# IDSIA/hhmarl_2D

Hardware: AMD Instinct MI355X
Metric: env-steps/sec (2v2) (higher is better)
Workload: dtype f64

## Files before the change

### hhmarl_2d_amd/csrc/hh_kernels_quad.h

```cpp
#ifndef HH_KERNELS_QUAD_H
#define HH_KERNELS_QUAD_H

#include "hh_kernels.h"

#define HH_QP(a, b, c, d) ((a) | ((b) << 2) | ((c) << 4) | ((d) << 6))

template <int CTRL>
__device__ __forceinline__ int q_perm_i(int v) { return __builtin_amdgcn_mov_dpp(v, CTRL, 0xf, 0xf, true); }
template <int CTRL>
__device__ __forceinline__ float q_perm_f(float v) { return __int_as_float(q_perm_i<CTRL>(__float_as_int(v))); }
template <int CTRL>
__device__ __forceinline__ double q_perm_d(double v) {
    int lo = __double2loint(v), hi = __double2hiint(v);
    lo = q_perm_i<CTRL>(lo);
    hi = q_perm_i<CTRL>(hi);
    return __hiloint2double(hi, lo);
}
#define HH_QROT(K) HH_QP((K) & 3, ((K) + 1) & 3, ((K) + 2) & 3, ((K) + 3) & 3)
template <int K> __device__ __forceinline__ int q_rot_i(int v) { return q_perm_i<HH_QROT(K)>(v); }
template <int K> __device__ __forceinline__ float q_rot_f(float v) { return q_perm_f<HH_QROT(K)>(v); }
template <int K> __device__ __forceinline__ double q_rot_d(double v) { return q_perm_d<HH_QROT(K)>(v); }
template <int J> __device__ __forceinline__ int q_bc_i(int v) { return q_perm_i<HH_QP(J, J, J, J)>(v); }
template <int J> __device__ __forceinline__ double q_bc_d(double v) { return q_perm_d<HH_QP(J, J, J, J)>(v); }
__device__ __forceinline__ double q_mate_d(double v) { return q_perm_d<HH_QP(1, 0, 3, 2)>(v); }
// ... 14 lines not shown

struct QPub {
    double uc, us, un;
    float nlat, nlon, nspd, nhdg;
    int flags;
};

struct QTab {
    double lat[3], lon[3];
    double dist[3], foc[3], focr[3], hd[3];
    float nlat[3], nlon[3], nspd[3], nhdg[3];
    int fl[3];
    int amask;
};

__device__ __forceinline__ void quad_publish_vec(const Unit &m, QPub &p) {
    double sn, cs;
    hh_sincos(hh_pymod360(90.0 - m.hdg) * (HH_PI / 180.0), &sn, &cs);
    p.uc = cs;
    p.us = sn;
    p.un = hh_sqrt(cs * cs + sn * sn);
}
__device__ __forceinline__ void quad_publish_norm(const DevCfg &c, const Unit &m, QPub &p) {
    p.nlat = (float)hh_clip(hh_div_known(m.lat - HH_MAP_LAT0, c.ext_lat, c.inv_ext_lat), 0.0, 1.0);
    p.nlon = (float)hh_clip(hh_div_known(m.lon - HH_MAP_LON0, c.ext_lon, c.inv_ext_lon), 0.0, 1.0);
    p.nspd = (float)hh_clip(hh_div_known(m.spd, HH_AC_MAX_SPEED(m.ac_type), HH_AC_INV_MAX_SPEED(m.ac_type)), 0.0, 1.0);
    p.nhdg = (float)hh_clip(HH_DIVC(hh_pymod359(m.hdg), 359.0), 0.0, 1.0);
}
__device__ __forceinline__ void quad_publish_motion(const DevCfg &c, const Unit &m, QPub &p) {
    quad_publish_vec(m, p);
    quad_publish_norm(c, m, p);
}

struct QPosMail { double lat[64], lon[64], spd[64], hdg[64]; int ac_type[64], steps[64], episode[64], escw[64]; };
struct QTabMail { double dist[3][64], foc[3][64], focr[3][64]; double uc[64], us[64], sx[64], sy[64]; unsigned long long tk[64];
                  double sp_hdg[64], sp_spd[64]; int sp_w[64];
                  double nr0[64], nfoc[64], nfocr[64]; int nbw[64]; };
struct QTgt { double foc, focr, dist; };
struct QSlimMail { int flags[64], w5[64], w6[64], w7[64]; double rew[64]; int full; };
struct QAheadMail { double u[2][64]; };
struct QPre {
    bool ok;
    bool a_ok;
    int a_par;
    bool spec;
    double sp_hdg, sp_spd;
    int sp_w;
    unsigned long long tkey;
    double sx, sy;
};
__device__ __forceinline__ void quad_publish_flags(const Unit &m, QPub &p) {
    int shot = m.burst > 0 || (m.ac_type == 1 && m.has_missile);
    p.flags = (m.alive ? FL_ALIVE : 0) | ((m.ac_type & 3) << 1) | (shot ? FL_SHOT : 0);
}
__device__ __forceinline__ void quad_publish(const DevCfg &c, const Unit &m, QPub &p) {
    quad_publish_motion(c, m, p);
    quad_publish_flags(m, p);
}

__device__ __forceinline__ void quad_tables_obs(const QPub &p, int s, QTab &t) {
#define HH_QFETCHO(K)                                                                 \
    t.nlat[K - 1] = q_rot_f<K>(p.nlat); t.nlon[K - 1] = q_rot_f<K>(p.nlon);               \
    t.nspd[K - 1] = q_rot_f<K>(p.nspd); t.nhdg[K - 1] = q_rot_f<K>(p.nhdg);               \
    t.fl[K - 1] = q_rot_i<K>(p.flags);
    HH_QFETCHO(1)
    HH_QFETCHO(2)
    HH_QFETCHO(3)
// ... 131 lines not shown
        }
        n += quad_opp_block(t, 0, nb.k0, nb.d0, out + n);
    } else {
        out[n++] = (float)hh_clip((double)m.cannon_remain / (double)m.cannon_max, 0.0, 1.0);
        if (m.ac_type == 1) out[n++] = (float)hh_clip((double)m.missile_remain / (double)m.rocket_max, 0.0, 1.0);
        out[n++] = (p.flags & FL_SHOT) ? 1.0f : 0.0f;
        quad_opp_block(t, 1, nb.k0, nb.d0, out + n);
        if (nb.n >= 2) quad_opp_block(t, 1, nb.k1, nb.d1, out + n + 9);
        else for (int k = 0; k < 9; k++) out[n + 9 + k] = 0.0f;
        n += 18;
    }
    const int kf = ((s ^ 1) - s) & 3;
    if ((t.amask >> (s ^ 1)) & 1) {
        out[n++] = q_sel(t.nlat, kf);
        out[n++] = q_sel(t.nlon, kf);
        out[n++] = (float)norm180(q_sel(t.foc, kf));
        out[n++] = (float)norm180(q_sel(t.focr, kf));
        out[n++] = (float)(c.inv_diag * q_sel(t.dist, kf));
    } else {
        for (int k = 0; k < 5; k++) out[n++] = 0.0f;
    }
}

__device__ __forceinline__ bool q_any(bool x) {
    unsigned long long b = __ballot(x);
    asm volatile("" : "+s"(b));
    return b != 0ULL;
}

__device__ __forceinline__ void arm_cannon_if(Unit &m, bool cond) {
    const int b = HH_AC_BURST(m.ac_type);
    const int armed = m.cannon_remain < b ? m.cannon_remain : b;
    m.burst = cond ? armed : m.burst;
}

__device__ __forceinline__ void q_wave_sync() { asm volatile("s_waitcnt lgkmcnt(0)" ::: "memory"); }

__device__ __forceinline__ void quad_l3_flags(int steps, unsigned long long tkey, int amask0, int s, int &esc, int &esc_t, bool &my_escaping, bool (&escj)[2]) {
    const bool draw_tick = steps % 60 == 0;
    const bool any_draw = q_any(draw_tick);
#pragma unroll
    for (int j = 2; j < 4; j++) {
        const bool aj = ((amask0 >> j) & 1) != 0;
        if (HH_RARE(any_draw)) {
            if (aj & draw_tick & (esc == 0)) {
                esc = hh_rng_randint(hh_rng_u01(tkey, (uint32_t)(j + 1), HH_SITE_L3_ESC_COIN, 0u), 0, 1);
                if (esc) esc_t = (int)hh_rng_uniform(hh_rng_u01(tkey, (uint32_t)(j + 1), HH_SITE_L3_ESC_TIME, 0u), 20.0, 30.0);
            }
        }
        const bool mine = aj & (j == s), upd = aj & (esc != 0);
        my_escaping = mine ? (esc != 0) : my_escaping;
        escj[j - 2] = aj & (esc != 0);
        const int esc_t1 = esc_t - 1;
        esc_t = upd ? esc_t1 : esc_t;
        esc = (upd & (esc_t <= 0)) ? 0 : esc;
    }
}
struct QScriptOut { double heading, speed; int fire, fire_m, opp; };
__device__ __forceinline__ void quad_l3_script(const DevCfg &c, double lat, double lon, double hdg, int ac_type, bool my_escaping, double u0, double u1, double u2,
                                               const Near2 &nb, const QTab &tb, double focus_k0, double rs, double rc, QScriptOut &o) {
    int opp = -1, fire = 0, fire_m = 0;
    double heading, speed;
    if (my_escaping) {
        double y = hh_clip(hh_div_known(lat - HH_MAP_LAT0, c.ext_lat, c.inv_ext_lat), 0.0, 1.0);
        double x = hh_clip(hh_div_known(lon - HH_MAP_LON0, c.ext_lon, c.inv_ext_lon), 0.0, 1.0);
        double uh = u0;
        double lo_h = y < 0.5 ? (x < 0.5 ? 30.0 : 300.0) : (x < 0.5 ? 120.0 : 210.0);
        heading = (double)(int)hh_rng_uniform(uh, lo_h, lo_h + 30.0);
        speed = (double)(int)hh_rng_uniform(u1, 300.0, 600.0);
        fire = hh_rng_randint(u2, 0, 1);
    } else {
        heading = hdg;
        speed = (double)(int)hh_rng_uniform(u0, 100.0, 400.0);
        if (nb.n) {
            const double ag_lat = q_sel(tb.lat, nb.k0), ag_lon = q_sel(tb.lon, nb.k0);
            double x1 = lon + rs, y1 = lat + rc;
            double val = (x1 - lon) * (ag_lat - lat) - (ag_lon - lon) * (y1 - lat);
            double sign = val < 0.0 ? 1.0 : -1.0;
            double r = hh_rng_uniform(u1, 0.7, 1.3);
            double focus = focus_k0;
            const double turned = hh_pymod360(heading + r * sign * focus);
            heading = ((nb.d0 > 0.008) & (focus > 4.0)) ? turned : heading;
            const double us = u2;
            const double sp_near = (double)(int)hh_rng_uniform(us, 500.0, 800.0), sp_far = (double)(int)hh_rng_uniform(us, 100.0, 500.0);
            const double sp2 = focus < 30.0 ? sp_near : sp_far;
            speed = nb.d0 > 0.05 ? sp2 : speed;
            fire = nb.d0 < 0.03 && focus < 10.0;
            fire_m = nb.d0 < 0.09 && focus < 5.0;
            opp = nb.j0;
        }
        if (ac_type == 2) speed = hh_clip(speed, 0.0, 600.0);
    }
    if (heading >= 360.0 || heading < 0.0) heading = 0.0;
    o.heading = heading; o.speed = speed; o.fire = fire; o.fire_m = fire_m; o.opp = opp;
}

template <bool IX, bool DUAL, bool OWT = false>
__device__ __forceinline__ void tick_quad(const DevCfg &c, Shared<4, 64> &sh, int tid, int g, int s, int base, bool active, bool helper, Unit &m,
                                          Arena &ar, const int8_t *act, QTab &tb, QPub &pub, Near2 &nbc, const QTgt &tg, StepOut &out,
                                          uint32_t &ev_mask_out, QPosMail *pos, const QAheadMail *ahd, const QPre &pre HH_PROF_ARGS) {
    constexpr int A = 4;
    const int id = s + 1;
    const bool running = active & (ar.done == 0);
    const bool agent = s < 2;
    out.reward = 0.0;
    out.valid = 0;
    out.kill_event = 0;
    uint32_t evm = 0;
    {
        const int steps1 = ar.steps + 1;
        ar.steps = running ? steps1 : ar.steps;
        if (OWT && HH_USUAL(pre.ok)) ar.tkey = running ? pre.tkey : ar.tkey;
        else if (running) arena_rekey(ar);
    }
    const bool snap = running & (m.alive != 0);
    const int amask0 = tb.amask;
    const int rk_age0 = (m.rk_alive && m.rk_life <= HH_ROCKET_MAX_LIFE) ? m.rk_life : 0;
    const double rk_speed0 = sh.rk_speed[rk_age0];
    const int tgt_at_act = m.n_tgt ? m.tgt0 : 0;
    int want_launch = 0, launch_tgt = 0;
    int wait_after = -1;
    bool base_gate = false;
    constexpr bool AHEAD = OWT && DUAL;
    double u_noise_ahead = 0.0;
    if constexpr (AHEAD) u_noise_ahead = ahd->u[pre.a_par][tid & 31];
    const bool a_ok = AHEAD && pre.a_ok;

    {
        if (HH_USUAL(snap & (agent | (c.ext_opp != 0)))) {
            int t = m.n_tgt ? m.tgt0 : 0;
            if (!agent) {
                const Near2 nb = nbc;
                m.n_tgt = nb.n ? 1 : 0; m.tgt0 = nb.n ? nb.j0 + 1 : 0; m.tgt_d0 = nb.n ? nb.d0 : 0.0;
                t = m.tgt0;
            }
            out.valid = agent ? 1 : out.valid;
#ifdef HHQ_ABL_DECODE
            m.cmd_hdg = m.hdg; m.cmd_spd = 300.0;
#else
            const double nh = hh_pymod360(m.hdg + (double)(((int)act[0] - 6) * 15));
            const bool nh_out = (nh >= 360.0) | (nh < 0.0);
            m.cmd_hdg = nh_out ? 0.0 : nh;
            double mx = HH_AC_MAX_SPEED(m.ac_type);
            m.cmd_spd = 100.0 + ((mx - 100.0) / 8.0) * (double)act[1];
#endif
            {
                const bool arm = (act[2] != 0) & (m.cannon_remain > 0);
                arm_cannon_if(m, arm);
                const double rw = out.reward - 0.1;
                const bool pen = arm & agent & (c.agent_mode == HH_MODE_ESCAPE) & (m.cannon_remain < 90);
                out.reward = pen ? rw : out.reward;
            }
            {
                const bool gate = (m.ac_type == 1) & (act[3] != 0) & (t != 0) & (m.missile_remain > 0) & (m.has_missile == 0) & (m.missile_wait == 0);
                base_gate = gate;
                want_launch = gate ? 1 : want_launch;
                launch_tgt = gate ? t - 1 : launch_tgt;
            }
        } else if (snap && c.level <= 2) {
            if (c.level == 2) {
                arm_cannon(m);
                bool man = ar.steps <= 5;
                if (!man) man = (ar.steps % hh_rng_randint(d_rng(ar, id, HH_SITE_L2_PERIOD, 0), 35, 45)) <= 5;
                if (man) {
                    int r = hh_rng_randint(d_rng(ar, id, HH_SITE_L2_TURN, 0), 0, 1);
                    m.cmd_hdg = hh_pymod360(m.hdg + (r ? -90.0 : 90.0));
                    m.cmd_spd = (double)(100 + hh_rng_randint(d_rng(ar, id, HH_SITE_L2_SPEED, 0), 0, 4) * 75);
                }
            }
            if (!m.has_missile && (ar.steps % 40) < 3 && hh_rng_randint(d_rng(ar, id, HH_SITE_L12_COIN, 0), 0, 1) &&
                m.missile_wait == 0 && m.ac_type == 1) {
                const Near2 nb = nbc;
                if (nb.n) { want_launch = 1; launch_tgt = nb.j0; wait_after = 5; }
            }
        }
    }
    HH_PROF(11);
    const bool spec = OWT && pre.ok && pre.spec && !c.ext_opp && c.level >= 3;
    bool my_escaping = false;
    bool escj[2] = {false, false};
    if (HH_RARE(!spec)) {
    if (HH_USUAL(running && !c.ext_opp && c.level >= 3)) {
        int esc = ar.escaping, esc_t = ar.escaping_time;
        quad_l3_flags(ar.steps, ar.tkey, amask0, s, esc, esc_t, my_escaping, escj);
        ar.escaping = esc;
        ar.escaping_time = esc_t;
    }
    double u0 = 0.0, u1 = 0.0, u2 = 0.0;
    if (!c.ext_opp && c.level >= 3) {
        {
            const int du = (s | 2) + 1;
            const bool desc = (s & 1) ? escj[1] : escj[0];
// ... 137 lines not shown
#else
            d_geo_move(x_lat, x_lon, x_hdg, x_s, o_lat, o_lon);
#endif
            m.lat = mv_a ? o_lat : m.lat; m.lon = mv_a ? o_lon : m.lon;
            rk_nlat = q_up_d(o_lat); rk_nlon = q_up_d(o_lon);
        } else if (HH_USUAL(any_rk)) {
            const double r_spd = rk_speed0;
            double a_lat, a_lon;
            d_geo_move2(m.lat, m.lon, m.hdg, mv_a ? m.spd * HH_KNOTS_TO_MS * 1.0 : 0.0, a_lat, a_lon,
                        rk_spec ? r_lat : 5.0, rk_spec ? r_lon : 7.0, r_hdg, r_spd * HH_KNOTS_TO_MS * 1.0, rk_nlat, rk_nlon);
            m.lat = mv_a ? a_lat : m.lat; m.lon = mv_a ? a_lon : m.lon;
        } else {
            if (mv_a) d_geo_move(m.lat, m.lon, m.hdg, m.spd * HH_KNOTS_TO_MS * 1.0, m.lat, m.lon);
        }
    }
    const double rk0_lat = rk_pre ? m.rk_lat : lat_old, rk0_lon = rk_pre ? m.rk_lon : lon_old;
    QPub pn;
    if constexpr (OWT) {
        {
            const double th = turn_deg * (HH_PI / 180.0), t2 = th * th;
            const double cd = 1.0 + t2 * (-0.5 + t2 * (1.0 / 24.0));
            const double sd = th * (1.0 + t2 * ((-1.0 / 6.0) + t2 * (1.0 / 120.0)));
            pn.uc = pub.uc * cd + pub.us * sd;
            pn.us = pub.us * cd - pub.uc * sd;
            pn.un = 1.0;
        }
        pn.nlat = pn.nlon = pn.nspd = pn.nhdg = 0.0f;
        pos->lat[tid] = m.lat;
        pos->lon[tid] = m.lon;
        pos->spd[tid] = m.spd; pos->hdg[tid] = m.hdg; pos->ac_type[tid] = m.ac_type;
        pos->steps[tid] = ar.steps; pos->episode[tid] = ar.episode;
        pos->escw[tid] = (ar.escaping & 0xff) | ((ar.escaping_time & 0xff) << 8) | ((amask0 & 0xf) << 16);
        HH_PROF(1);
        __syncthreads();
        HH_PROF(12);
    } else {
        quad_publish_motion(c, m, pn);
    }
    double lat1[3], lon1[3];
    lat1[0] = q_rot_d<1>(m.lat); lon1[0] = q_rot_d<1>(m.lon);
    lat1[1] = q_rot_d<2>(m.lat); lon1[1] = q_rot_d<2>(m.lon);
    lat1[2] = q_rot_d<3>(m.lat); lon1[2] = q_rot_d<3>(m.lon);

    HH_PROF(1);
    const int rk_tgt = rk_pre ? m.rk_target - 1 : launch_tgt;
    const bool rk_maybe = running && (rk_pre || try_launch);
    int launch_pre = -1;
    if (q_any(try_launch)) {
        const int kl = (launch_tgt - s) & 3;
        const double t_lat = q_sel(tb.lat, kl), t_lon = q_sel(tb.lon, kl);
        const double cross = pub.uc * (t_lat - lat_old) - pub.us * (t_lon - lon_old);
        const int lp = hh_missile_cone_planar(lat_old, lon_old, t_lat, t_lon, OWT ? tg.foc : q_sel(tb.foc, kl), cross, OWT ? tg.dist : q_sel(tb.dist, kl));
        launch_pre = try_launch ? lp : -1;
    }
    int q_total = 0;
    {
        int push[6];
        int code[6];
        push[0] = try_launch && launch_pre < 0;
        code[0] = tid | (0 << 8) | (launch_tgt << 10);
        const int t = m.ac_type;
#pragma unroll
        for (int k = 1; k < A; k++) {
            const int j = (s + k) & 3;
            const bool snap_j = running && ((amask0 >> j) & 1);
            const bool enemy = (j >= 2) != (s >= 2);
            const double tl = j < s ? lat1[k - 1] : tb.lat[k - 1];
// ... 3 lines not shown
#else
            push[k] = (int)fired & (int)snap_j & ((int)(c.friendly_kill != 0) | (int)enemy) & (int)d_maybe_within_km(lat_old, lon_old, tl, to, HH_AC_CANNON_KM(t)) &
                      (int)!hh_cannon_cone_planar_outside(lat_old, lon_old, tl, to, pn.uc, pn.us, t);
#endif
            code[k] = tid | (1 << 8) | (j << 10);
        }
        {
            const int kt = (rk_tgt - s) & 3;
            const double tl = kt ? q_sel(lat1, kt) : m.lat, to = kt ? q_sel(lon1, kt) : m.lon;
            push[4] = (int)rk_maybe & (int)d_maybe_within_km(rk0_lat, rk0_lon, tl, to, HH_ROCKET_FUSE_KM);
            code[4] = tid | (2 << 8) | (rk_tgt << 10);
            const int fid = s == 1 ? 0 : 1;
            const int kf = (fid - s) & 3;
            const double fl_ = kf ? q_sel(lat1, kf) : m.lat, fo_ = kf ? q_sel(lon1, kf) : m.lon;
            push[5] = (int)rk_maybe & (int)(c.friendly_kill != 0) & (int)d_maybe_within_km(rk0_lat, rk0_lon, fl_, fo_, HH_ROCKET_FUSE_KM);
            code[5] = tid | (3 << 8) | (fid << 10);
        }
        if (HH_RARE(__ballot(push[0] | push[1] | push[2] | push[3] | push[4] | push[5]) != 0ULL)) {
#pragma unroll
            for (int e = 0; e < 6; e++) {
                const unsigned long long bm = __ballot(push[e]);
                if (push[e]) {
                    int pos = q_total + (int)__builtin_amdgcn_mbcnt_hi((unsigned)(bm >> 32), __builtin_amdgcn_mbcnt_lo((unsigned)bm, 0u));
                    sh.u.t.q_code[pos] = code[e];
                }
                q_total += __popcll(bm);
#ifdef HH_PROFILE_PHASES
                if (tid == 0 && bm) atomicAdd(&hh_prof_cycles[e == 0 ? 13 : (e < 4 ? 14 : 15)], (unsigned long long)__popcll(bm));
#endif
            }
        }
#ifdef HH_PROFILE_PHASES
        if (tid == 0 && q_total) atomicAdd(&hh_prof_cycles[12], 1ULL);
#endif
    }
    HH_PROF(2);
    int myres = 0;
    if (HH_RARE(q_total != 0)) {
        sh.lat0[tid] = lat_old; sh.lon0[tid] = lon_old; sh.hdg[tid] = hdg_old;
        sh.flags[tid] = pub.flags;
        sh.u.t.lat1[tid] = m.lat; sh.u.t.lon1[tid] = m.lon; sh.u.t.hdg1[tid] = m.hdg;
        sh.u.t.rk_lat[tid] = rk0_lat; sh.u.t.rk_lon[tid] = rk0_lon;
        sh.res[tid] = 0;
        if (s == 0 && !helper) sh.g_tkey[g] = ar.tkey;
        q_wave_sync();
        drain_envelope_queue<4, 64, IX>(sh, tid, q_total);
        q_wave_sync();
        myres = sh.res[tid];
    }
    if (launch_pre == 1) myres |= 1;

    HH_PROF(3);
    int launched = 0;
    const bool launch_now = try_launch & ((myres & 1) != 0);
    if (q_any(launch_now)) if (launch_now) {
        launched = 1;
        m.rk_alive = 1; m.rk_lat = lat_old; m.rk_lon = lon_old; m.rk_hdg = hdg_old;
        m.rk_target = launch_tgt + 1; m.rk_life = 0;
        m.has_missile = 1;
        m.missile_remain = m.missile_remain - 1 > 0 ? m.missile_remain - 1 : 0;
        evm |= 1u << (24 + s);
        m.rk_cmd = rk_ncmd;
    }
    if (q_any(base_gate)) if (base_gate) {
        double uu;
        if (HH_USUAL(a_ok)) uu = ahd->u[pre.a_par][32 + (tid & 31)];
// ... 293 lines not shown
        DevCfg d = c;
        hh_cfg_set_preset(d, pre);
        if (d.level == c.level && d.agent_mode == c.agent_mode && d.ext_opp == c.ext_opp && d.friendly_kill == c.friendly_kill &&
            d.friendly_punish == c.friendly_punish && d.esc_dist_rew == c.esc_dist_rew && d.glob_frac == c.glob_frac && d.rew_scale == c.rew_scale &&
            d.D == c.D && d.n_ctrl == c.n_ctrl && d.nA == c.nA && d.nO == c.nO)
            return pre;
    }
    return 0;
}
template <int W, int PRE, bool TWO, int APW = 16, bool DUAL = false, bool SHAPE = true>
__global__ __launch_bounds__(TWO ? 128 : 64, W) __attribute__((amdgpu_waves_per_eu(W, W))) void hh_k_world_quad(DevPtrs P, DevCfg c_in, int T, const int8_t *__restrict__ actions,
                                                                  float *__restrict__ obs_out, float *__restrict__ reward_out,
                                                                  uint8_t *__restrict__ valid_out, uint8_t *__restrict__ done_out) {
    constexpr int A = 4, B = 64, GPB = APW;
    static_assert(APW == 16 || APW == 8, "arenas per wave");
    static_assert(!DUAL || APW == 8, "helper lanes exist only where half the wave is idle");
    DevCfg c_pre = c_in;
    hh_cfg_set_preset(c_pre, PRE);
    const DevCfg &c = PRE ? c_pre : c_in;
    __shared__ Shared<A, B> sh;
    __shared__ QuadMailbox<TWO> mbx;
    const int tid = threadIdx.x & 63;
    const int D = c.D;
    static_assert(SHAPE || (PRE == 0 && TWO), "SHAPE = false names the general two-wave instance without escape shaping");
    constexpr bool OWT = TWO && (PRE != 0 || !SHAPE);
    if constexpr (OWT) {
        if (threadIdx.x >= 64) {
            const bool helper = DUAL && tid >= 32;
            const int mt = DUAL ? (tid & 31) : tid;
            const int g = mt >> 2, s = mt & 3;
            const int n = blockIdx.x * GPB + g;
            const bool row = !helper && s < 2 && g < GPB && n < c.N;
#ifdef HH_PROFILE_PHASES
            unsigned long long ot0_ = __builtin_readcyclecounter(), oacc_[4] = {0, 0, 0, 0};
#define HH_OPROF(k) do { unsigned long long t_ = __builtin_readcyclecounter(); oacc_[k] += t_ - ot0_; ot0_ = t_; } while (0)
#else
#define HH_OPROF(k)
#endif
            const unsigned long long akey = hh_rng_arena_key(c.seed, c.arena_offset + (uint64_t)n);
            const bool stat_lane = row && s == 0;
            double ep_ret = stat_lane ? P.ep_ret[n] : 0.0;
            for (int t = 0; t < T; t++) {
                __syncthreads();
                HH_OPROF(0);
                Unit m = Unit{};
                QPub pub;
                m.lat = mbx.pos.lat[tid]; m.lon = mbx.pos.lon[tid]; m.spd = mbx.pos.spd[tid]; m.hdg = mbx.pos.hdg[tid];
                m.ac_type = mbx.pos.ac_type[tid];
                pub.flags = 0;
                double rs_ahead = 0.0, rc_ahead = 0.0;
                if constexpr (DUAL) {
                    const double hmain = q_down_d(m.hdg);
                    double sn, cs;
                    hh_sincos((helper ? hh_pymod360(hmain) : hh_pymod360(90.0 - hmain)) * (HH_PI / 180.0), &sn, &cs);
                    pub.uc = cs; pub.us = sn; pub.un = hh_sqrt(cs * cs + sn * sn);
                    rs_ahead = q_up_d(hh_round3(sn)); rc_ahead = q_up_d(hh_round3(cs));
                } else {
                    quad_publish_vec(m, pub);
                    double sn, cs;
                    hh_sincos(hh_pymod360(m.hdg) * (HH_PI / 180.0), &sn, &cs);
                    rs_ahead = hh_round3(sn); rc_ahead = hh_round3(cs);
                }
                const int steps_t = mbx.pos.steps[mt];
                const int episode_t = mbx.pos.episode[mt];
                const unsigned long long tk1 = hh_rng_tick_key(akey, (uint32_t)episode_t, (uint32_t)(steps_t + 1));
                const bool l3 = !c.ext_opp && c.level >= 3;
                const int ew = mbx.pos.escw[mt];
                int esc = ew & 0xff, esc_t = (int)(int8_t)((ew >> 8) & 0xff);
                const int am = (ew >> 16) & 0xf;
                bool my_escaping = false, escj[2] = {false, false};
                double u0 = 0.0, u1 = 0.0, u2 = 0.0;
                if (l3) {
                    quad_l3_flags(steps_t + 1, tk1, am, s, esc, esc_t, my_escaping, escj);
                    const int du = (s | 2) + 1, role = helper ? 2 : (s < 2 ? 1 : 0);
                    const int site_e = role == 0 ? HH_SITE_ESC_HDG : (role == 1 ? HH_SITE_ESC_SPEED : HH_SITE_ESC_FIRE);
                    const int site_h = role == 0 ? HH_SITE_HC_SPEED1 : (role == 1 ? HH_SITE_HC_R : HH_SITE_HC_SPEED2);
                    const bool desc = (s & 1) ? escj[1] : escj[0];
                    int de = desc ? 1 : 0;
                    if (DUAL) { const int deh = q_down_i(de); de = helper ? deh : de; }
                    const double u = hh_rng_u01(tk1, (uint32_t)du, (uint32_t)(de ? site_e : site_h), 0u);
                    u0 = u; u1 = q_perm_d<HH_QP(0, 1, 0, 1)>(u);
                    if (DUAL) u2 = q_up_d(u);
                    else u2 = hh_rng_u01(tk1, (uint32_t)(s + 1), (uint32_t)(my_escaping ? HH_SITE_ESC_FIRE : HH_SITE_HC_SPEED2), 0u);
                }
                QTab tb;
                quad_tables<DUAL, false>(m, pub, s, helper, tb);
#pragma unroll
                for (int k = 0; k < 3; k++) { mbx.tab.dist[k][tid] = tb.dist[k]; mbx.tab.foc[k][tid] = tb.foc[k]; mbx.tab.focr[k][tid] = tb.focr[k]; }
                mbx.tab.uc[tid] = pub.uc; mbx.tab.us[tid] = pub.us;
                mbx.tab.tk[tid] = tk1;
                mbx.tab.sx[tid] = rs_ahead; mbx.tab.sy[tid] = rc_ahead;
                tb.amask = am;
                Near2 nb;
                quad_nearby(c, tb, s, nb);
                const double foc_k0 = q_sel(tb.foc, nb.k0);
                mbx.tab.nr0[tid] = nb.r0; mbx.tab.nfoc[tid] = foc_k0; mbx.tab.nfocr[tid] = q_sel(tb.focr, nb.k0);
                mbx.tab.nbw[tid] = (nb.n & 3) | ((nb.j0 & 3) << 2) | ((nb.k0 & 3) << 4);
                if (l3) {
                    QScriptOut so_;
                    quad_l3_script(c, m.lat, m.lon, m.hdg, m.ac_type, my_escaping, u0, u1, u2, nb, tb, foc_k0, rs_ahead, rc_ahead, so_);
                    mbx.tab.sp_hdg[tid] = so_.heading; mbx.tab.sp_spd[tid] = so_.speed;
                    mbx.tab.sp_w[tid] = (so_.fire & 1) | ((so_.fire_m & 1) << 1) | (((so_.opp + 1) & 7) << 2) | ((esc & 0xff) << 8) | ((esc_t & 0xff) << 16);
                }
                HH_OPROF(1);
                __syncthreads();
                HH_OPROF(2);
                int valid = 0, done = 0;
                float rew = 0.0f;
                {
                    const int w7s = mbx.slim.w7[tid];
                    const double rv = ((w7s >> 24) & 1) ? mbx.slim.rew[tid] : 0.0;
                    const double r1 = q_rot_d<1>(rv);
                    const bool ran = ((w7s >> 26) & 1) != 0, dn = ((w7s >> 25) & 1) != 0;
                    const double e2 = (ep_ret + rv) + r1;
                    ep_ret = ran ? e2 : ep_ret;
                    if (HH_RARE(stat_lane && ran && dn)) {
                        const int am = (w7s >> 27) & 0xf, steps = steps_t;
                        const int ag = __popc(am & 3), op = __popc(am & 12);
                        P.last_ret[n] = (float)ep_ret;
                        P.last_len[n] = steps;
                        P.last_outcome[n] = (op <= 0 && steps < c.horizon) ? 1 : ((ag <= 0 && steps < c.horizon) ? -1 : 0);
                    }
                    if (dn && c.auto_reset) ep_ret = 0.0;
                }
                if (HH_RARE(mbx.slim.full)) {
                    if (row) mail_take(mbx.mail[0], g * 2 + s, tb, pub, m, valid, done, rew);
                } else {
                    pub.flags = mbx.slim.flags[tid];
                    quad_publish_norm(c, m, pub);
                    quad_tables_obs(pub, s, tb);
                    const int w5 = mbx.slim.w5[tid], w6 = mbx.slim.w6[tid], w7 = mbx.slim.w7[tid];
                    m.cannon_remain = w5 & 0xffff; m.cannon_max = (w5 >> 16) & 0xffff;
                    m.missile_remain = w6 & 0xff; m.rocket_max = (w6 >> 8) & 0xff; m.missile_wait = (w6 >> 16) & 0xff; m.burst = (w6 >> 24) & 0xff;
                    m.ac_type = w7 & 0xff; m.alive = (w7 >> 8) & 0xff; m.has_missile = (w7 >> 16) & 0xff;
                    valid = (w7 >> 24) & 1;
                    done = (w7 >> 25) & 1;
                    rew = (float)mbx.slim.rew[tid];
                }
                if (HH_USUAL(row)) {
                    quad_lowlevel_obs(c, tb, pub, s, c.agent_mode, m, &mbx.tile[(g * 2 + s) * D], D);
                    const size_t o = ((size_t)t * c.N + n) * 2 + s;
                    if (reward_out) reward_out[o] = rew;
                    if (valid_out) valid_out[o] = (uint8_t)valid;
                    if (s == 0 && done_out) done_out[(size_t)t * c.N + n] = (uint8_t)done;
                }
                q_wave_sync();
                if (obs_out) quad_store_rows<GPB>(obs_out, mbx.tile, t, c.N, D, tid);
                if constexpr (DUAL) {
                    int steps_2 = steps_t + 2;
                    asm volatile("" : "+v"(steps_2));
                    const unsigned long long tk2 = hh_rng_tick_key(akey, (uint32_t)episode_t, (uint32_t)steps_2);
                    mbx.ahead.u[t & 1][tid] = hh_rng_u01(tk2, (uint32_t)(s + 1), (uint32_t)(helper ? HH_SITE_MISSILE_WAIT : HH_SITE_ROCKET_NOISE), 0u);
                }
                q_wave_sync();
                HH_OPROF(3);
            }
            if (stat_lane) P.ep_ret[n] = ep_ret;
#ifdef HH_PROFILE_PHASES
            if (tid == 0) for (int k_ = 0; k_ < 4; k_++) atomicAdd(&hh_prof_cycles[16 + k_], oacc_[k_]);
#endif
#undef HH_OPROF
            return;
        }
    } else if constexpr (TWO) {
        if (threadIdx.x >= 64) {
            const int g = tid >> 1, s = tid & 1;
            const int n = blockIdx.x * GPB + g;
            const bool row = tid < 2 * GPB && n < c.N;
            for (int t = 0; t < T; t++) {
                __syncthreads();
                const ObsMail &mb = mbx.mail[t & 1];
                if (row) {
                    QTab tb; QPub pub; Unit m;
                    int valid, done; float rew;
                    mail_take(mb, tid, tb, pub, m, valid, done, rew);
                    quad_lowlevel_obs(c, tb, pub, s, c.agent_mode, m, &mbx.tile[tid * D], D);
                    const size_t o = ((size_t)t * c.N + n) * 2 + s;
                    if (reward_out) reward_out[o] = rew;
                    if (valid_out) valid_out[o] = (uint8_t)valid;
                    if (s == 0 && done_out) done_out[(size_t)t * c.N + n] = (uint8_t)done;
                }
                q_wave_sync();
                if (obs_out) quad_store_rows<GPB>(obs_out, mbx.tile, t, c.N, D, tid);
                q_wave_sync();
            }
            return;
        }
    }
    const bool helper = DUAL && tid >= 32;
    const int mt = DUAL ? (tid & 31) : tid;
    const int g = mt >> 2, s = mt & 3;
    const int base = g * A;
    const int n = blockIdx.x * GPB + g;
    const bool active = !helper && g < GPB && n < c.N;
    const size_t U = (size_t)c.N * A;
    const size_t u = (size_t)n * A + s;
    HH_PROF_DECL;
    Unit m = Unit{};
    Arena ar = Arena{};
    double ep_ret = 0.0;
    if (active) {
        unit_load(P, U, u, m);
        arena_load(P, c, n, ar);
        ep_ret = P.ep_ret[n];
    } else {
        ar.done = 1;
    }
    uint32_t evm_last = 0;
    int act_fault = 0;
    {
        const double speed_table[11] = HH_ROCKET_SPEED_TABLE;
        if (tid < 11) sh.rk_speed[tid] = speed_table[tid];
    }
    QPub pub;
    QTab tb;
    Near2 nbc;
    quad_publish(c, m, pub);
    quad_tables<DUAL>(m, pub, s, helper, tb);
    quad_nearby(c, tb, s, nbc);
    QTgt tg;
    {
        const int ks = (s < 2 && m.n_tgt) ? ((m.tgt0 - 1 - s) & 3) : nbc.k0;
        tg.foc = q_sel(tb.foc, ks); tg.focr = q_sel(tb.focr, ks); tg.dist = q_sel(tb.dist, ks);
    }
    const bool has_act = active && s < c.n_ctrl;
    QPre pre;
    pre.ok = false; pre.spec = false; pre.sp_hdg = pre.sp_spd = 0.0; pre.sp_w = 0;
    pre.tkey = 0ULL; pre.sx = pre.sy = 0.0;
    pre.a_ok = false; pre.a_par = 0;
    double inv_diag_v = c.inv_diag;
    if constexpr (OWT) asm volatile("" : "+v"(inv_diag_v));
    bool noreset_prev = false;
    const size_t act_stride = (size_t)c.N * c.n_ctrl * 4;
    const int8_t *act_ptr = has_act ? actions + ((size_t)n * c.n_ctrl + s) * 4 : actions;
    int act_cur = *reinterpret_cast<const int *>(act_ptr);
    int act_next = *reinterpret_cast<const int *>(act_ptr + (size_t)min(1, T - 1) * act_stride);
    q_wave_sync();
    for (int t = 0; t < T; t++) {
        StepOut so;
        int8_t act[4];
        const bool was_running = active && !ar.done;
        hh_act_unpack(act_cur, act, act_fault, has_act & was_running & (m.alive != 0));
        QPosMail *posmail = nullptr;
        const QAheadMail *ahdmail = nullptr;
        if constexpr (OWT) { posmail = &mbx.pos; ahdmail = &mbx.ahead; }
        const int amask_before = tb.amask;
        tick_quad<(W >= 2), DUAL, OWT>(c, sh, tid, g, s, base, active, helper, m, ar, act, tb, pub, nbc, tg, so, evm_last, posmail, ahdmail, pre HH_PROF_PASS);
        const int done_now = ar.done;
        if constexpr (TWO && !OWT) {
            if (!helper && s < 2) mail_post(mbx.mail[t & 1], g * 2 + s, tb, pub, m, so, done_now);
        }
        asm volatile("" : "+v"(act_next));
        act_cur = act_next;
        act_next = *reinterpret_cast<const int *>(act_ptr + (size_t)min(t + 2, T - 1) * act_stride);
        if (!TWO && HH_USUAL(active && s < 2)) {
            size_t o = ((size_t)t * c.N + n) * 2 + s;
            if (reward_out) reward_out[o] = (float)so.reward;
            if (valid_out) valid_out[o] = (uint8_t)so.valid;
        }
        const int amask_stats = tb.amask;
        if constexpr (!OWT) {
            const double rv = so.valid ? so.reward : 0.0;
            const double r0 = q_bc_d<0>(rv), r1 = q_bc_d<1>(rv);
            {
                const double e2 = (ep_ret + r0) + r1;
                ep_ret = was_running ? e2 : ep_ret;
                const bool fin = was_running & (ar.done != 0) & (s == 0);
                if (HH_RARE(q_any(fin))) if (fin) {
                    const int ag = __popc(tb.amask & 3), op = __popc(tb.amask & 12);
                    P.last_ret[n] = (float)ep_ret;
                    P.last_len[n] = ar.steps;
                    P.last_outcome[n] = (op <= 0 && ar.steps < c.horizon) ? 1 : ((ag <= 0 && ar.steps < c.horizon) ? -1 : 0);
                }
            }
        }
        if (!TWO && active && s == 0 && done_out) done_out[(size_t)t * c.N + n] = (uint8_t)ar.done;
        const bool need_reset = active && ar.done && c.auto_reset;
        const bool reset_tick = q_any(need_reset);
        if (HH_RARE(reset_tick)) {
            if (need_reset) {
                reset_arena_scalars(ar);
                reset_unit<A>(c, s, m, ar);
                ep_ret = 0.0;
            }
            quad_publish(c, m, pub);
            quad_tables<DUAL>(m, pub, s, helper, tb);
            quad_nearby(c, tb, s, nbc);
            tg.foc = q_sel(tb.foc, nbc.k0); tg.focr = q_sel(tb.focr, nbc.k0); tg.dist = nbc.r0;
            if constexpr (OWT) {
                if (!helper && s < 2) mail_post(mbx.mail[0], g * 2 + s, tb, pub, m, so, done_now);
            } else if constexpr (TWO) {
                if (!helper && s < 2) mail_post(mbx.mail[t & 1], g * 2 + s, tb, pub, m, so, done_now);
            }
        }
        HH_PROF(9);
        if constexpr (OWT) {
            mbx.slim.flags[tid] = pub.flags;
            mbx.slim.w5[tid] = (m.cannon_remain & 0xffff) | ((m.cannon_max & 0xffff) << 16);
            mbx.slim.w6[tid] = (m.missile_remain & 0xff) | ((m.rocket_max & 0xff) << 8) | ((m.missile_wait & 0xff) << 16) | ((m.burst & 0xff) << 24);
            mbx.slim.w7[tid] = (m.ac_type & 0xff) | ((m.alive & 0xff) << 8) | ((m.has_missile & 0xff) << 16) | ((so.valid & 1) << 24) | ((done_now & 1) << 25) |
                               ((was_running ? 1 : 0) << 26) | ((amask_stats & 0xf) << 27);
            mbx.slim.rew[tid] = so.reward;
            if (tid == 0) mbx.slim.full = reset_tick ? 1 : 0;
            HH_PROF(9);
            __syncthreads();
            HH_PROF(13);
            const unsigned long long m_tk = mbx.tab.tk[tid];
            const double m_sx = mbx.tab.sx[tid], m_sy = mbx.tab.sy[tid], m_uc = mbx.tab.uc[tid], m_us = mbx.tab.us[tid];
            const double m_sp_hdg = mbx.tab.sp_hdg[tid], m_sp_spd = mbx.tab.sp_spd[tid];
            const int m_sp_w = mbx.tab.sp_w[tid], m_nbw = mbx.tab.nbw[tid];
            const double m_nr0 = mbx.tab.nr0[tid], m_nfoc = mbx.tab.nfoc[tid], m_nfocr = mbx.tab.nfocr[tid];
            pre.ok = !reset_tick;
            pre.a_ok = !reset_tick && noreset_prev;
            noreset_prev = !reset_tick;
            pre.a_par = (t + 1) & 1;
            pre.spec = !reset_tick && !q_any(active && tb.amask != amask_before);
            if (HH_USUAL(!reset_tick)) {
                pre.tkey = m_tk; pre.sx = m_sx; pre.sy = m_sy;
                pub.uc = m_uc; pub.us = m_us;
                pre.sp_hdg = m_sp_hdg; pre.sp_spd = m_sp_spd; pre.sp_w = m_sp_w;
                if (HH_USUAL(pre.spec)) {
                    const int w = m_nbw;
                    const double r0 = m_nr0;
                    tg.foc = m_nfoc; tg.focr = m_nfocr; tg.dist = r0;
                    nbc.n = w & 3; nbc.j0 = (w >> 2) & 3; nbc.k0 = (w >> 4) & 3;
                    nbc.r0 = r0; nbc.d0 = inv_diag_v * r0;
                    nbc.j1 = nbc.k1 = 0; nbc.d1 = nbc.r1 = 0.0;
                } else {
                    QTab tf = tb;
#pragma unroll
                    for (int k = 0; k < 3; k++) { tf.dist[k] = mbx.tab.dist[k][tid]; tf.foc[k] = mbx.tab.foc[k][tid]; tf.focr[k] = mbx.tab.focr[k][tid]; }
                    quad_nearby(c, tf, s, nbc);
                    tg.foc = q_sel(tf.foc, nbc.k0); tg.focr = q_sel(tf.focr, nbc.k0); tg.dist = nbc.r0;
                }
            }
            {
                Unit mr = m;
                quad_target_refresh(nbc, mr);
                const bool keep = active & (s < 2);
                m.n_tgt = keep ? mr.n_tgt : m.n_tgt; m.tgt0 = keep ? mr.tgt0 : m.tgt0; m.tgt_d0 = keep ? mr.tgt_d0 : m.tgt_d0;
            }
            HH_PROF(10);
            continue;
        } else if constexpr (TWO) {
            {
                Unit mr = m;
                quad_target_refresh(nbc, mr);
                const bool keep = active & (s < 2);
                m.n_tgt = keep ? mr.n_tgt : m.n_tgt; m.tgt0 = keep ? mr.tgt0 : m.tgt0; m.tgt_d0 = keep ? mr.tgt_d0 : m.tgt_d0;
            }
            __syncthreads();
            HH_PROF(10);
            continue;
        }
        if (HH_USUAL(active && s < 2)) quad_lowlevel_obs(c, tb, pub, s, c.agent_mode, m, &sh.u.obs[(g * 2 + s) * D], D);
        q_wave_sync();
        if (obs_out) quad_store_rows<GPB>(obs_out, sh.u.obs, t, c.N, D, tid);
        q_wave_sync();
        HH_PROF(10);
    }
    HH_PROF_FLUSH;
    if (active) {
        unit_store(P, U, u, m);
        if (s == 0) {
            arena_store(P, n, ar);
            if constexpr (!OWT) P.ep_ret[n] = ep_ret;
            P.ev_mask[n] = 0;
        }
    }
    q_wave_sync();
    if (active && evm_last) atomicOr(&P.ev_mask[n], evm_last);
    hh_act_fault_commit(P, n, active, act_fault);
}

#endif
```

Before: 965.3 million.

## Decode next-step actions ahead and carry precomputed RNG draws in helper warp

In the OWT path, the action word for the next tick is decoded into a QCmd (heading, speed, arm/launch bits) before the barrier, so the tick body no longer unpacks and decodes actions on its critical path. The helper/opponent loop now caches the next tick key and the two escape/heuristic uniform draws computed one step ahead, and reuses them when the episode/step match, skipping the hash recomputation. Profiling counters per tick class are added under HH_PROFILE_PHASES. This adds registers and live state across barriers, and depends on the carried values staying consistent with the mailbox step/episode.

```diff
diff --git a/hhmarl_2d_amd/csrc/hh_kernels_quad.h b/hhmarl_2d_amd/csrc/hh_kernels_quad.h
--- a/hhmarl_2d_amd/csrc/hh_kernels_quad.h
+++ b/hhmarl_2d_amd/csrc/hh_kernels_quad.h
@@ -70,7 +70,20 @@
     quad_publish_norm(c, m, p);
 }
 
-struct QPosMail { double lat[64], lon[64], spd[64], hdg[64]; int ac_type[64], steps[64], episode[64], escw[64]; };
+#ifdef HH_PROFILE_PHASES
+__device__ unsigned long long hh_prof_class[24];
+extern "C" int hh_prof_class_read(unsigned long long *out24, int reset) {
+    if (hipDeviceSynchronize() != hipSuccess) return -1;
+    if (hipMemcpyFromSymbol(out24, HIP_SYMBOL(hh_prof_class), 24 * 8) != hipSuccess) return -1;
+    if (reset) { unsigned long long z[24] = {0}; if (hipMemcpyToSymbol(HIP_SYMBOL(hh_prof_class), z, 24 * 8) != hipSuccess) return -1; }
+    return 0;
+}
+#define HH_PROF_CLS_ADD(acc, base, cls, v) do { _Pragma("unroll") for (int k_ = 0; k_ < 4; k_++) (acc)[(base) + k_] += (cls) == k_ ? (unsigned long long)(v) : 0ULL; } while (0)
+#define HH_PROF_CLS_WORDS int prof_q, prof_cls; unsigned long long prof_tx[2];
+#else
+#define HH_PROF_CLS_WORDS
+#endif
+struct QPosMail { double lat[64], lon[64], spd[64], hdg[64]; int ac_type[64], steps[64], episode[64], escw[64]; HH_PROF_CLS_WORDS };
 struct QTabMail { double dist[3][64], foc[3][64], focr[3][64]; double uc[64], us[64], sx[64], sy[64]; unsigned long long tk[64];
                   double sp_hdg[64], sp_spd[64]; int sp_w[64];
                   double nr0[64], nfoc[64], nfocr[64]; int nbw[64]; };
@@ -268,6 +281,28 @@
     const int b = HH_AC_BURST(m.ac_type);
     const int armed = m.cannon_remain < b ? m.cannon_remain : b;
     m.burst = cond ? armed : m.burst;
+}
+
+struct QCmd { double hdg, spd; bool arm, launch; };
+__device__ __forceinline__ void quad_decode_parts(const int8_t (&act)[4], const Unit &m, QCmd &o) {
+#ifdef HHQ_ABL_DECODE
+    o.hdg = m.hdg; o.spd = 300.0;
+#else
+    const double nh = hh_pymod360(m.hdg + (double)(((int)act[0] - 6) * 15));
+    const bool nh_out = (nh >= 360.0) | (nh < 0.0);
+    o.hdg = nh_out ? 0.0 : nh;
+    double mx = HH_AC_MAX_SPEED(m.ac_type);
+    o.spd = 100.0 + ((mx - 100.0) / 8.0) * (double)act[1];
+#endif
+    o.arm = (act[2] != 0) & (m.cannon_remain > 0);
+    o.launch = act[3] != 0;
+}
+__device__ __forceinline__ int quad_decode_cmd(int word, const Unit &m, bool consumed, QCmd &o) {
+    int8_t act[4];
+    int fault = 0;
+    hh_act_unpack(word, act, fault, consumed);
+    quad_decode_parts(act, m, o);
+    return fault;
 }
 
 __device__ __forceinline__ void q_wave_sync() { asm volatile("s_waitcnt lgkmcnt(0)" ::: "memory"); }
@@ -333,7 +368,7 @@
 
 template <bool IX, bool DUAL, bool OWT = false>
 __device__ __forceinline__ void tick_quad(const DevCfg &c, Shared<4, 64> &sh, int tid, int g, int s, int base, bool active, bool helper, Unit &m,
-                                          Arena &ar, const int8_t *act, QTab &tb, QPub &pub, Near2 &nbc, const QTgt &tg, StepOut &out,
+                                          Arena &ar, const int8_t (&act)[4], const QCmd &cmd_ahead, QTab &tb, QPub &pub, Near2 &nbc, const QTgt &tg, StepOut &out,
                                           uint32_t &ev_mask_out, QPosMail *pos, const QAheadMail *ahd, const QPre &pre HH_PROF_ARGS) {
     constexpr int A = 4;
     const int id = s + 1;
@@ -362,8 +397,36 @@
     if constexpr (AHEAD) u_noise_ahead = ahd->u[pre.a_par][tid & 31];
     const bool a_ok = AHEAD && pre.a_ok;
 
+    const bool acts = snap & (agent | (c.ext_opp != 0));
+    if constexpr (OWT) {
+        int t = m.n_tgt ? m.tgt0 : 0;
+        if (c.ext_opp) {
+            const Near2 nb = nbc;
+            const bool rf = acts & !agent;
+            const int nt = nb.n ? 1 : 0, t0 = nb.n ? nb.j0 + 1 : 0;
+            const double d0 = nb.n ? nb.d0 : 0.0;
+            m.n_tgt = rf ? nt : m.n_tgt; m.tgt0 = rf ? t0 : m.tgt0; m.tgt_d0 = rf ? d0 : m.tgt_d0;
+            t = rf ? t0 : t;
+        }
+        out.valid = (acts & agent) ? 1 : out.valid;
+        m.cmd_hdg = acts ? cmd_ahead.hdg : m.cmd_hdg;
+        m.cmd_spd = acts ? cmd_ahead.spd : m.cmd_spd;
+        {
+            const bool arm = acts & cmd_ahead.arm;
+            arm_cannon_if(m, arm);
+            const double rw = out.reward - 0.1;
+            const bool pen = arm & agent & (c.agent_mode == HH_MODE_ESCAPE) & (m.cannon_remain < 90);
+            out.reward = pen ? rw : out.reward;
+        }
+        {
+            const bool gate = acts & (m.ac_type == 1) & cmd_ahead.launch & (t != 0) & (m.missile_remain > 0) & (m.has_missile == 0) & (m.missile_wait == 0);
+            base_gate = gate;
+            want_launch = gate ? 1 : want_launch;
+            launch_tgt = gate ? t - 1 : launch_tgt;
+        }
+    }
     {
-        if (HH_USUAL(snap & (agent | (c.ext_opp != 0)))) {
+        if (!OWT && HH_USUAL(acts)) {
             int t = m.n_tgt ? m.tgt0 : 0;
             if (!agent) {
                 const Near2 nb = nbc;
@@ -371,29 +434,24 @@
                 t = m.tgt0;
             }
             out.valid = agent ? 1 : out.valid;
-#ifdef HHQ_ABL_DECODE
-            m.cmd_hdg = m.hdg; m.cmd_spd = 300.0;
-#else
-            const double nh = hh_pymod360(m.hdg + (double)(((int)act[0] - 6) * 15));
-            const bool nh_out = (nh >= 360.0) | (nh < 0.0);
-            m.cmd_hdg = nh_out ? 0.0 : nh;
-            double mx = HH_AC_MAX_SPEED(m.ac_type);
-            m.cmd_spd = 100.0 + ((mx - 100.0) / 8.0) * (double)act[1];
-#endif
+            QCmd cmd;
+            quad_decode_parts(act, m, cmd);
+            m.cmd_hdg = cmd.hdg;
+            m.cmd_spd = cmd.spd;
             {
-                const bool arm = (act[2] != 0) & (m.cannon_remain > 0);
+                const bool arm = cmd.arm;
                 arm_cannon_if(m, arm);
                 const double rw = out.reward - 0.1;
                 const bool pen = arm & agent & (c.agent_mode == HH_MODE_ESCAPE) & (m.cannon_remain < 90);
                 out.reward = pen ? rw : out.reward;
             }
             {
-                const bool gate = (m.ac_type == 1) & (act[3] != 0) & (t != 0) & (m.missile_remain > 0) & (m.has_missile == 0) & (m.missile_wait == 0);
+                const bool gate = (m.ac_type == 1) & cmd.launch & (t != 0) & (m.missile_remain > 0) & (m.has_missile == 0) & (m.missile_wait == 0);
                 base_gate = gate;
                 want_launch = gate ? 1 : want_launch;
                 launch_tgt = gate ? t - 1 : launch_tgt;
             }
-        } else if (snap && c.level <= 2) {
+        } else if (snap && c.level <= 2 && !(OWT && acts)) {
             if (c.level == 2) {
                 arm_cannon(m);
                 bool man = ar.steps <= 5;
@@ -597,7 +655,13 @@
         pos->steps[tid] = ar.steps; pos->episode[tid] = ar.episode;
         pos->escw[tid] = (ar.escaping & 0xff) | ((ar.escaping_time & 0xff) << 8) | ((amask0 & 0xf) << 16);
         HH_PROF(1);
+#ifdef HH_PROFILE_PHASES
+        if (tid == 0) pos->prof_tx[0] = __builtin_readcyclecounter();
+#endif
         __syncthreads();
+#ifdef HH_PROFILE_PHASES
+        if (tid == 0) pos->prof_tx[1] = __builtin_readcyclecounter();
+#endif
         HH_PROF(12);
     } else {
         quad_publish_motion(c, m, pn);
@@ -667,6 +731,7 @@
         }
 #ifdef HH_PROFILE_PHASES
         if (tid == 0 && q_total) atomicAdd(&hh_prof_cycles[12], 1ULL);
+        if constexpr (OWT) { if (tid == 0) pos->prof_q = (q_total != 0 ? 2 : 0) | (spec ? 0 : 1); }
 #endif
     }
     HH_PROF(2);
@@ -1026,7 +1091,7 @@
             const int n = blockIdx.x * GPB + g;
             const bool row = !helper && s < 2 && g < GPB && n < c.N;
 #ifdef HH_PROFILE_PHASES
-            unsigned long long ot0_ = __builtin_readcyclecounter(), oacc_[4] = {0, 0, 0, 0};
+            unsigned long long ot0_ = __builtin_readcyclecounter(), oacc_[4] = {0, 0, 0, 0}, ocls_[8] = {0}, oprev_[2] = {0, 0};
 #define HH_OPROF(k) do { unsigned long long t_ = __builtin_readcyclecounter(); oacc_[k] += t_ - ot0_; ot0_ = t_; } while (0)
 #else
 #define HH_OPROF(k)
@@ -1034,6 +1099,13 @@
             const unsigned long long akey = hh_rng_arena_key(c.seed, c.arena_offset + (uint64_t)n);
             const bool stat_lane = row && s == 0;
             double ep_ret = stat_lane ? P.ep_ret[n] : 0.0;
+            const int du = (s | 2) + 1, role = helper ? 2 : (s < 2 ? 1 : 0);
+            const int site_e = role == 0 ? HH_SITE_ESC_HDG : (role == 1 ? HH_SITE_ESC_SPEED : HH_SITE_ESC_FIRE);
+            const int site_h = role == 0 ? HH_SITE_HC_SPEED1 : (role == 1 ? HH_SITE_HC_R : HH_SITE_HC_SPEED2);
+            unsigned long long c_tk = 0ULL;
+            double c_ue = 0.0, c_uh = 0.0;
+            int c_ep = 0, c_st = 0;
+            const bool has_arena = n < c.N;
             for (int t = 0; t < T; t++) {
                 __syncthreads();
                 HH_OPROF(0);
@@ -1057,7 +1129,15 @@
                 }
                 const int steps_t = mbx.pos.steps[mt];
                 const int episode_t = mbx.pos.episode[mt];
-                const unsigned long long tk1 = hh_rng_tick_key(akey, (uint32_t)episode_t, (uint32_t)(steps_t + 1));
+                bool carried = false;
+                if constexpr (DUAL) carried = !q_any(has_arena & ((episode_t != c_ep) | (steps_t + 1 != c_st)));
+                unsigned long long tk1;
+                if (DUAL && HH_USUAL(carried)) tk1 = c_tk;
+                else {
+                    int steps_1 = steps_t + 1;
+                    if constexpr (DUAL) asm volatile("" : "+v"(steps_1));
+                    tk1 = hh_rng_tick_key(akey, (uint32_t)episode_t, (uint32_t)steps_1);
+                }
                 const bool l3 = !c.ext_opp && c.level >= 3;
                 const int ew = mbx.pos.escw[mt];
                 int esc = ew & 0xff, esc_t = (int)(int8_t)((ew >> 8) & 0xff);
@@ -1066,13 +1146,16 @@
                 double u0 = 0.0, u1 = 0.0, u2 = 0.0;
                 if (l3) {
                     quad_l3_flags(steps_t + 1, tk1, am, s, esc, esc_t, my_escaping, escj);
-                    const int du = (s | 2) + 1, role = helper ? 2 : (s < 2 ? 1 : 0);
-                    const int site_e = role == 0 ? HH_SITE_ESC_HDG : (role == 1 ? HH_SITE_ESC_SPEED : HH_SITE_ESC_FIRE);
-                    const int site_h = role == 0 ? HH_SITE_HC_SPEED1 : (role == 1 ? HH_SITE_HC_R : HH_SITE_HC_SPEED2);
                     const bool desc = (s & 1) ? escj[1] : escj[0];
                     int de = desc ? 1 : 0;
                     if (DUAL) { const int deh = q_down_i(de); de = helper ? deh : de; }
-                    const double u = hh_rng_u01(tk1, (uint32_t)du, (uint32_t)(de ? site_e : site_h), 0u);
+                    double u;
+                    if (DUAL && HH_USUAL(carried)) u = de ? c_ue : c_uh;
+                    else {
+                        int site = de ? site_e : site_h;
+                        if constexpr (DUAL) asm volatile("" : "+v"(site));
+                        u = hh_rng_u01(tk1, (uint32_t)du, (uint32_t)site, 0u);
+                    }
                     u0 = u; u1 = q_perm_d<HH_QP(0, 1, 0, 1)>(u);
                     if (DUAL) u2 = q_up_d(u);
                     else u2 = hh_rng_u01(tk1, (uint32_t)(s + 1), (uint32_t)(my_escaping ? HH_SITE_ESC_FIRE : HH_SITE_HC_SPEED2), 0u);
@@ -1099,6 +1182,13 @@
                 HH_OPROF(1);
                 __syncthreads();
                 HH_OPROF(2);
+#ifdef HH_PROFILE_PHASES
+                {
+                    const int cls_ = mbx.pos.prof_cls;
+                    HH_PROF_CLS_ADD(ocls_, 0, cls_, oacc_[1] - oprev_[0]); HH_PROF_CLS_ADD(ocls_, 4, cls_, oacc_[2] - oprev_[1]);
+                    oprev_[0] = oacc_[1]; oprev_[1] = oacc_[2];
+                }
+#endif
                 int valid = 0, done = 0;
                 float rew = 0.0f;
                 {
@@ -1145,6 +1235,11 @@
                     asm volatile("" : "+v"(steps_2));
                     const unsigned long long tk2 = hh_rng_tick_key(akey, (uint32_t)episode_t, (uint32_t)steps_2);
                     mbx.ahead.u[t & 1][tid] = hh_rng_u01(tk2, (uint32_t)(s + 1), (uint32_t)(helper ? HH_SITE_MISSILE_WAIT : HH_SITE_ROCKET_NOISE), 0u);
+                    c_tk = tk2;
+                    c_ue = hh_rng_u01(tk2, (uint32_t)du, (uint32_t)site_e, 0u);
+                    c_uh = hh_rng_u01(tk2, (uint32_t)du, (uint32_t)site_h, 0u);
+                    c_ep = episode_t; c_st = steps_2;
+                    asm volatile("" : "+v"(c_tk), "+v"(c_ue), "+v"(c_uh));
                 }
                 q_wave_sync();
                 HH_OPROF(3);
@@ -1152,6 +1247,7 @@
             if (stat_lane) P.ep_ret[n] = ep_ret;
 #ifdef HH_PROFILE_PHASES
             if (tid == 0) for (int k_ = 0; k_ < 4; k_++) atomicAdd(&hh_prof_cycles[16 + k_], oacc_[k_]);
+            if (tid == 0) for (int k_ = 0; k_ < 8; k_++) atomicAdd(&hh_prof_class[8 + k_], ocls_[k_]);
 #endif
 #undef HH_OPROF
             return;
@@ -1190,6 +1286,9 @@
     const size_t U = (size_t)c.N * A;
     const size_t u = (size_t)n * A + s;
     HH_PROF_DECL;
+#ifdef HH_PROFILE_PHASES
+    unsigned long long scls_[16] = {0}, sym_ = __builtin_readcyclecounter();
+#endif
     Unit m = Unit{};
     Arena ar = Arena{};
     double ep_ret = 0.0;
@@ -1230,16 +1329,28 @@
     int act_cur = *reinterpret_cast<const int *>(act_ptr);
     int act_next = *reinterpret_cast<const int *>(act_ptr + (size_t)min(1, T - 1) * act_stride);
     q_wave_sync();
+    QCmd cmd_ahead;
+    cmd_ahead.hdg = cmd_ahead.spd = 0.0; cmd_ahead.arm = cmd_ahead.launch = false;
+    int cmd_bits = 0;
+    if constexpr (OWT) {
+        const int f0 = quad_decode_cmd(act_cur, m, has_act & (active && !ar.done) & (m.alive != 0) & (T > 0), cmd_ahead);
+        act_fault |= f0;
+        cmd_bits = (cmd_ahead.arm ? 1 : 0) | (cmd_ahead.launch ? 2 : 0);
+    }
+#ifdef HH_PROFILE_PHASES
+    sym_ = __builtin_readcyclecounter();
+#endif
     for (int t = 0; t < T; t++) {
         StepOut so;
         int8_t act[4];
         const bool was_running = active && !ar.done;
-        hh_act_unpack(act_cur, act, act_fault, has_act & was_running & (m.alive != 0));
+        if constexpr (!OWT) hh_act_unpack(act_cur, act, act_fault, has_act & was_running & (m.alive != 0));
+        else { cmd_ahead.arm = (cmd_bits & 1) != 0; cmd_ahead.launch = (cmd_bits & 2) != 0; }
         QPosMail *posmail = nullptr;
         const QAheadMail *ahdmail = nullptr;
         if constexpr (OWT) { posmail = &mbx.pos; ahdmail = &mbx.ahead; }
         const int amask_before = tb.amask;
-        tick_quad<(W >= 2), DUAL, OWT>(c, sh, tid, g, s, base, active, helper, m, ar, act, tb, pub, nbc, tg, so, evm_last, posmail, ahdmail, pre HH_PROF_PASS);
+        tick_quad<(W >= 2), DUAL, OWT>(c, sh, tid, g, s, base, active, helper, m, ar, act, cmd_ahead, tb, pub, nbc, tg, so, evm_last, posmail, ahdmail, pre HH_PROF_PASS);
         const int done_now = ar.done;
         if constexpr (TWO && !OWT) {
             if (!helper && s < 2) mail_post(mbx.mail[t & 1], g * 2 + s, tb, pub, m, so, done_now);
@@ -1296,8 +1407,31 @@
                                ((was_running ? 1 : 0) << 26) | ((amask_stats & 0xf) << 27);
             mbx.slim.rew[tid] = so.reward;
             if (tid == 0) mbx.slim.full = reset_tick ? 1 : 0;
+            {
+                int w_next = act_cur;
+                asm volatile("" : "+v"(w_next) : : "memory");
+                const int f1 = quad_decode_cmd(w_next, m, has_act & (active && !ar.done) & (m.alive != 0) & (t + 1 < T), cmd_ahead);
+                act_fault |= f1;
+                cmd_bits = (cmd_ahead.arm ? 1 : 0) | (cmd_ahead.launch ? 2 : 0);
+                asm volatile("" : "+v"(cmd_ahead.hdg), "+v"(cmd_ahead.spd), "+v"(cmd_bits));
+            }
             HH_PROF(9);
+#ifdef HH_PROFILE_PHASES
+            const int cls_ = reset_tick ? 3 : ((mbx.pos.prof_q & 2) ? 2 : (mbx.pos.prof_q & 1));
+            if (tid == 0) mbx.pos.prof_cls = cls_;
+            const unsigned long long sxm_ = mbx.pos.prof_tx[0], sxa_ = mbx.pos.prof_tx[1];
+            const unsigned long long cy0_ = __builtin_readcyclecounter();
+#endif
             __syncthreads();
+#ifdef HH_PROFILE_PHASES
+            {
+                const unsigned long long cy1_ = __builtin_readcyclecounter();
+                HH_PROF_CLS_ADD(scls_, 0, cls_, 1); HH_PROF_CLS_ADD(scls_, 4, cls_, cy1_ - cy0_);
+                HH_PROF_CLS_ADD(scls_, 8, cls_, sxm_ - sym_);
+                HH_PROF_CLS_ADD(scls_, 12, cls_, cy0_ - sxa_);
+                sym_ = cy1_;
+            }
+#endif
             HH_PROF(13);
             const unsigned long long m_tk = mbx.tab.tk[tid];
             const double m_sx = mbx.tab.sx[tid], m_sy = mbx.tab.sy[tid], m_uc = mbx.tab.uc[tid], m_us = mbx.tab.us[tid];
@@ -1354,6 +1488,12 @@
         HH_PROF(10);
     }
     HH_PROF_FLUSH;
+#ifdef HH_PROFILE_PHASES
+    if constexpr (OWT) if (tid == 0) {
+        for (int k_ = 0; k_ < 8; k_++) atomicAdd(&hh_prof_class[k_], scls_[k_]);
+        for (int k_ = 0; k_ < 8; k_++) atomicAdd(&hh_prof_class[16 + k_], scls_[8 + k_]);
+    }
+#endif
     if (active) {
         unit_store(P, U, u, m);
         if (s == 0) {
```

Result: no change. 973.6 million, median of 6 (+0.9%).
